# smallflyingpig/speech-to-image-translation-without-text

Measured on AMD Instinct MI355X. Metric: StackGAN-v2 3-stage G+D train-step images/sec at 256px, higher is better.
Workload: dtype f32

## Files before the change

### include/s2i_hip.h

```cpp
#ifndef S2I_HIP_H
#define S2I_HIP_H

#include <stddef.h>
#include <stdint.h>

#ifdef __cplusplus
extern "C" {
#endif

#define S2I_ABI_VERSION 7

#define S2I_CONV_K1      0
#define S2I_CONV_K3S1    1
#define S2I_CONV_K4S2    2
#define S2I_TCONV_K4S2   3

#define S2I_CONV_1D      4

#define S2I_ACT_NONE     0
#define S2I_ACT_GLU      1
#define S2I_ACT_LRELU    2
#define S2I_ACT_TANH     3
#define S2I_ACT_RELU     4

// ... 93 lines not shown


int s2i_conv_bf16_plan_query(const s2i_conv_desc* d, long long out[21]);
int s2i_pack_conv_weight_bf16(const s2i_conv_desc* d, const float* packed, int R, int C, unsigned short* out,
                              void* stream);
typedef struct s2i_pack16_item {
  const float* P;
  unsigned short* out;
  int R, C, kind, flip, transpose, T, nphase, Nn, Npad, Kk, CK, gx, gy, block0;
} s2i_pack16_item;
int s2i_pack16_item_fill(const s2i_conv_desc* d, const float* packed, int R, int C, unsigned short* out,
                         s2i_pack16_item* item);
int s2i_pack_conv_weights_bf16_batched(const s2i_pack16_item* items_dev, int n, int total_blocks, void* stream);
int s2i_conv_forward_bf16(const s2i_conv_desc* d, const unsigned short* x, const unsigned short* w,
                          const float* cls_bias, unsigned short* y, float* part, void* ws, size_t ws_bytes,
                          void* stream);
int s2i_conv_forward_dt(const s2i_conv_desc* d, const void* x, int x_dtype, const float* cvec, const float* w,
                        const float* bias, const float* cls_bias, void* y, int y_dtype, float* part, void* ws,
                        size_t ws_bytes, void* stream);
size_t s2i_wgrad_workspace_bytes_dt(const s2i_wgrad_desc* d, int a_dtype, int g_dtype);
int s2i_wgrad_plan_query(const s2i_wgrad_desc* d, int a_dtype, int g_dtype, int planes, int in_act, int out[12]);
int s2i_conv_wgrad_dt(const s2i_wgrad_desc* d, const void* a, int a_dtype, const float* cvec, const void* g,
                      int g_dtype, float* grad_oihw, void* ws, size_t ws_bytes, void* stream);
int s2i_bn_act_forward_dt(int dtype, const void* y, long long M, int groups, int C, const float* coef4, int act,
                          const void* residual, void* out, void* stream);
int s2i_bn_act_bwd_reduce_dt(int dtype, const void* y, const void* dout, int lddout, long long M, int groups, int C,
                             const float* coef4, int act, float* part, int nparts, void* stream);
int s2i_bn_act_bwd_apply_dt(int dtype, const void* y, const void* dout, int lddout, long long M, int groups, int C,
                            const float* coef4, const float* red2, int act, void* dy, void* stream);
int s2i_act_backward_dt(int dtype, const void* out, const void* dout, int lddout, long long M, int C, int act,
                        void* dy, void* stream);
int s2i_nchw_to_nhwc_dt(int dtype, const float* src, void* dst, int B, int C, int H, int W, int Cp, void* stream);
int s2i_nhwc_to_nchw_dt(int dtype, const void* src, int lds, float* dst, int B, int C, int H, int W, void* stream);
int s2i_spatial_sum_dt(int dtype, const void* src, int ld, int B, int HW, int C, float* dst, void* ws,
                       size_t ws_bytes, void* stream);
int s2i_tap_sums_dt(int dtype, const void* dy, int B, int H, int W, int C, float* tapsum, void* ws, size_t ws_bytes,
                    void* stream);
int s2i_cast(const void* src, int src_dtype, void* dst, int dst_dtype, long long n, void* stream);

int s2i_pack_conv_weight(const float* w_oihw, float* packed, int O, int I, int KH, int KW,
                         int Ip, int mode, void* stream);
typedef struct s2i_pack_item {
  const float* w;
  float* packed;
  int O, I, KH, KW, Ip, mode, gx, block0;
} s2i_pack_item;
// ... 227 lines not shown
```

### speech_to_image_translation_without_text_amd/_lib.py

```python
import ctypes
import os

import torch

_HERE = os.path.dirname(os.path.abspath(__file__))
LIB_PATH = os.path.join(_HERE, "libs2i_hip.so")

CONV_K1, CONV_K3S1, CONV_K4S2, TCONV_K4S2, CONV_1D = 0, 1, 2, 3, 4
ACT_NONE, ACT_GLU, ACT_LRELU, ACT_TANH, ACT_RELU = 0, 1, 2, 3, 4
PACK_PLAIN, PACK_UPFOLD = 0, 1
DT_F32, DT_BF16 = 0, 1
POOL_MAX3S2, POOL_AVG3S1, POOL_GLOBAL = 0, 1, 2
POOL_THEN_LRN, LRN_THEN_POOL = 0, 1
LOGMEL_BFT, LOGMEL_NHWC = 0, 1
ENC_LOSS_JEL, ENC_LOSS_L1, ENC_LOSS_DISTILL = 1, 2, 4
LOGMEL_TILE_FRAMES = 64
PCM_U8, PCM_S16, PCM_S24, PCM_S32, PCM_F32, PCM_F64 = 0, 1, 2, 3, 4, 5
RESAMPLE_TILE = 1024
RESAMPLE_MAX_WINDOW = 13826
TOPK_MAX = 64
RANK_GATHER, RANK_COUNT = 0, 1
DIFFAUG_COLOR, DIFFAUG_TRANSLATION, DIFFAUG_CUTOUT = 1, 2, 4
ABI_VERSION = 7
WGRAD_KERNELS = ("f32-128x128", "f32-128x64", "f32-128x32", "f32-64x64", "f32-256x128", "f32-256x256", "f32-96x64", "f32-96x32",
# ... 24 lines not shown
                                     "tile_rows", "in_act", "in_groups")]


class Conv2dDesc(ctypes.Structure):
    _fields_ = [(n, c_int) for n in ("B", "H", "W", "C", "ldx", "N", "kh", "kw", "sh", "sw", "ph", "pw", "Ho", "Wo",
                                     "ldy", "coff", "relu", "tile")]


class WgradDesc(ctypes.Structure):
    _fields_ = [(n, c_int) for n in ("kind", "B", "H", "W", "Ca", "Cc", "N", "ldg", "swap", "fold",
                                     "O", "I", "KH", "KW", "accumulate", "i_off", "I_total", "a_act", "a_groups")]


class PackItem(ctypes.Structure):
    _fields_ = [("w", c_void_p), ("packed", c_void_p)] + [(n, c_int) for n in ("O", "I", "KH", "KW", "Ip", "mode", "gx",
                                                                               "block0")]


class Pack16Item(ctypes.Structure):
    _fields_ = [("P", c_void_p), ("out", c_void_p)] + [(n, c_int) for n in (
        "R", "C", "kind", "flip", "transpose", "T", "nphase", "Nn", "Npad", "Kk", "CK", "gx", "gy", "block0")]


P = c_void_p
_SIGNATURES = {
    "s2i_last_error": (ctypes.c_char_p, []),
    "s2i_version": (c_int, []),
    "s2i_check_device": (c_int, []),
    "s2i_set_tuning": (c_int, [ctypes.c_char_p, c_int]),
    "s2i_get_tuning": (c_int, [ctypes.c_char_p, ctypes.POINTER(c_int)]),
    "s2i_conv_workspace_bytes": (c_size_t, [ctypes.POINTER(ConvDesc)]),
    "s2i_conv_stat_parts": (c_int, [ctypes.POINTER(ConvDesc)]),
    "s2i_conv_plan_query": (c_int, [ctypes.POINTER(ConvDesc), c_int, c_int, c_int, c_int, c_int, ctypes.POINTER(c_int * 15)]),
    "s2i_conv_forward": (c_int, [ctypes.POINTER(ConvDesc), P, P, P, P, P, P, P, c_size_t, P]),
    "s2i_conv_forward_cls": (c_int, [ctypes.POINTER(ConvDesc), P, P, P, P, P, P, P, P, c_size_t, P]),
    "s2i_conv_forward_in": (c_int, [ctypes.POINTER(ConvDesc), P, P, P, P, P, P, c_size_t, P]),
    "s2i_conv_wgrad_in_eligible": (c_int, [ctypes.POINTER(WgradDesc)]),
    "s2i_conv_wgrad_in": (c_int, [ctypes.POINTER(WgradDesc), P, P, P, P, P, c_size_t, P]),
    "s2i_conv_split_eligible": (c_int, [ctypes.POINTER(ConvDesc)]),
    "s2i_conv_forward_split": (c_int, [ctypes.POINTER(ConvDesc), P, P, P, c_int, c_int, c_int, P, P, P, P, P, c_size_t, P]),
    "s2i_split_packed_weight": (c_int, [P, c_int, c_int, c_int, c_int, P, P, P]),
    "s2i_wgrad_workspace_bytes_split": (c_size_t, [ctypes.POINTER(WgradDesc), c_int]),
    "s2i_conv_wgrad_split": (c_int, [ctypes.POINTER(WgradDesc), c_int, P, P, P, P, P, c_size_t, P]),
    "s2i_conv_bf16_plan_query": (c_int, [ctypes.POINTER(ConvDesc), ctypes.POINTER(c_ll * 21)]),
    "s2i_pack16_item_fill": (c_int, [ctypes.POINTER(ConvDesc), P, c_int, c_int, P, ctypes.POINTER(Pack16Item)]),
    "s2i_pack_conv_weights_bf16_batched": (c_int, [P, c_int, c_int, P]),
    "s2i_pack_conv_weight_bf16": (c_int, [ctypes.POINTER(ConvDesc), P, c_int, c_int, P, P]),
    "s2i_conv_forward_bf16": (c_int, [ctypes.POINTER(ConvDesc), P, P, P, P, P, P, c_size_t, P]),
    "s2i_conv_forward_dt": (c_int, [ctypes.POINTER(ConvDesc), P, c_int, P, P, P, P, P, c_int, P, P, c_size_t, P]),
    "s2i_wgrad_workspace_bytes_dt": (c_size_t, [ctypes.POINTER(WgradDesc), c_int, c_int]),
    "s2i_conv_wgrad_dt": (c_int, [ctypes.POINTER(WgradDesc), P, c_int, P, P, c_int, P, P, c_size_t, P]),
    "s2i_wgrad_plan_query": (c_int, [ctypes.POINTER(WgradDesc), c_int, c_int, c_int, c_int, ctypes.POINTER(c_int * 12)]),
    "s2i_bn_act_forward_dt": (c_int, [c_int, P, c_ll, c_int, c_int, P, c_int, P, P, P]),
    "s2i_bn_act_bwd_reduce_dt": (c_int, [c_int, P, P, c_int, c_ll, c_int, c_int, P, c_int, P, c_int, P]),
    "s2i_bn_act_bwd_apply_dt": (c_int, [c_int, P, P, c_int, c_ll, c_int, c_int, P, P, c_int, P, P]),
    "s2i_act_backward_dt": (c_int, [c_int, P, P, c_int, c_ll, c_int, c_int, P, P]),
    "s2i_nchw_to_nhwc_dt": (c_int, [c_int, P, P, c_int, c_int, c_int, c_int, c_int, P]),
    "s2i_nhwc_to_nchw_dt": (c_int, [c_int, P, c_int, P, c_int, c_int, c_int, c_int, P]),
    "s2i_spatial_sum_dt": (c_int, [c_int, P, c_int, c_int, c_int, c_int, P, P, c_size_t, P]),
    "s2i_tap_sums_dt": (c_int, [c_int, P, c_int, c_int, c_int, c_int, P, P, c_size_t, P]),
    "s2i_cast": (c_int, [P, c_int, P, c_int, c_ll, P]),
    "s2i_cvec_bias_table": (c_int, [P, P, c_int, c_int, c_int, c_int, c_int, P, P, c_size_t, P]),
    "s2i_border_sums_workspace_bytes": (c_size_t, [c_int, c_int, c_int, c_int]),
    "s2i_tap_sums": (c_int, [P, c_int, c_int, c_int, c_int, P, P, c_size_t, P]),
    "s2i_cvec_grads": (c_int, [P, P, P, c_int, c_int, c_int, c_int, c_int, c_int, c_int, P, P, c_int, P]),
    "s2i_wgrad_workspace_bytes": (c_size_t, [ctypes.POINTER(WgradDesc)]),
    "s2i_conv_wgrad": (c_int, [ctypes.POINTER(WgradDesc), P, P, P, P, P, c_size_t, P]),
    "s2i_pack_conv_weight": (c_int, [P, P, c_int, c_int, c_int, c_int, c_int, c_int, P]),
    "s2i_pack_conv_weights_batched": (c_int, [P, c_int, c_int, c_int, P]),
    "s2i_bn_finalize": (c_int, [P, c_int, c_int, c_int, c_ll, P, P, P, P, P, c_float, c_float, P, P]),
    "s2i_bn_eval_coeffs": (c_int, [c_int, P, P, P, P, c_float, P, P]),
    "s2i_bn_act_forward": (c_int, [P, c_ll, c_int, c_int, P, c_int, P, P, P]),
    "s2i_colstats": (c_int, [P, c_ll, c_int, c_int, P, c_int, P]),
    "s2i_bn_act_bwd_reduce": (c_int, [P, P, c_int, c_ll, c_int, c_int, P, c_int, P, c_int, P]),
    "s2i_bn_bwd_finalize": (c_int, [P, c_int, c_int, c_int, c_ll, P, P, c_int, P, P]),
# ... 195 lines not shown
```

### speech_to_image_translation_without_text_amd/csrc/s2i_wgrad.hip

```cpp
#include "s2i_igemm.h"

namespace {

struct WgradP {
  const float* __restrict__ a;
  const float* __restrict__ cvec;
  const float* __restrict__ g;
  float* __restrict__ slab;
  int B, H, W, Ca, Cc, Cin;
  int Ho, Wo, lgWo, lgHoWo;
  int M, N, ldg, K, T, kind;
  int cps, nchunks;
  int a16, g16;
  unsigned a_bytes, c_bytes, g_bytes;
  const float* __restrict__ a_coef;
  int a_groups, a_ipg;
};

__device__ __forceinline__ bool wgrad_col(const WgradP& p, int kcol, int kw, int& c, int& dy, int& dx) {
  c = 0;
  dy = 0;
  dx = 0;
  if (kcol >= p.K) return false;
  const int t = kcol / p.Cin;
// ... 540 lines not shown
    const f32x4 av0 = load_a(m0);
    load_g(m0, g0);
    fma9(av0, g0);
  }
#pragma unroll
  for (int t = 0; t < 9; ++t)
#pragma unroll
    for (int j = 0; j < 4; ++j) {
      f32x4 v = acc[t][j];
#pragma unroll
      for (int sft = LPP; sft < 64; sft <<= 1)
#pragma unroll
        for (int n = 0; n < 4; ++n) v[n] += __shfl_xor(v[n], sft);
      if (pl == 0) red[wave][(t * LPP + q) * 4 + j] = v;
    }
  __syncthreads();
  float* outp = p.slab + (size_t)blockIdx.x * p.K * 4;
  for (int e = tid; e < 9 * LPP * 4; e += 256) {
    const f32x4 v = red[0][e] + red[1][e] + red[2][e] + red[3][e];
    *reinterpret_cast<f32x4*>(outp + (size_t)e * 4) = v;
  }
}

__global__ __launch_bounds__(256) void slab_sum_tree_kernel(float* __restrict__ slab, int S, int n4) {
  __shared__ f32x4 sh[256];
  const int tid = threadIdx.x;
  const int e = blockIdx.x * 4 + (tid & 3), sl = tid >> 2;
  f32x4 v = {0.f, 0.f, 0.f, 0.f};
  if (e < n4)
    for (int s = sl; s < S; s += 64) v += *reinterpret_cast<const f32x4*>(slab + ((size_t)s * n4 + e) * 4);
  sh[tid] = v;
  __syncthreads();
  for (int h = 32; h >= 1; h >>= 1) {
    if (sl < h) sh[tid] += sh[tid + h * 4];
    __syncthreads();
  }
  if (sl == 0 && e < n4) *reinterpret_cast<f32x4*>(slab + (size_t)e * 4) = sh[tid];
}

__global__ __launch_bounds__(256) void slab_sum_kernel(float* __restrict__ slab, int S, long long n4) {
  for (long long e = (long long)blockIdx.x * blockDim.x + threadIdx.x; e < n4;
       e += (long long)gridDim.x * blockDim.x) {
    f32x4 v = *reinterpret_cast<const f32x4*>(slab + e * 4);
    for (int s = 1; s < S; ++s) v += *reinterpret_cast<const f32x4*>(slab + ((size_t)s * n4 + e) * 4);
    *reinterpret_cast<f32x4*>(slab + e * 4) = v;
  }
}

__global__ __launch_bounds__(256) void wgrad_finish_kernel(const float* __restrict__ slab, int S, int K, int N,
                                                           int Cg, int O, int I, int Tp, int T, int swap, int fold,
                                                           int accumulate, int RT, float* __restrict__ grad,
                                                           int i_off, int I_total) {
  extern __shared__ float tile[];
  const int tid = threadIdx.x;
  const int ncols = swap ? I : O, nrows = swap ? O : I;
  const int c0 = blockIdx.x * 32, r0 = blockIdx.y * RT;
  const size_t sstride = (size_t)K * N;
  const int nload = T * RT * 32;
  for (int e = tid; e < nload; e += 256) {
    const int c_l = e & 31;
    const int r_l = (e >> 5) % RT;
    const int t = (e >> 5) / RT;
    const int c = c0 + c_l, r = r0 + r_l;
    float v = 0.f;
    if (c < ncols && r < nrows) {
      const float* sp = slab + ((size_t)t * Cg + r) * N + c;
      for (int s = 0; s < S; ++s) v += sp[s * sstride];
    }
    tile[(t * RT + r_l) * 33 + c_l] = v;
  }
  __syncthreads();
  const int nout = 32 * RT * Tp;
  for (int w = tid; w < nout; w += 256) {
    const int tapo = w % Tp;
    const int rest = w / Tp;
    int o_l, i_l, r_l, c_l;
    if (swap) { i_l = rest & 31; o_l = rest >> 5; r_l = o_l; c_l = i_l; }
    else { i_l = rest % RT; o_l = rest / RT; r_l = i_l; c_l = o_l; }
    const int o = swap ? r0 + o_l : c0 + o_l;
    const int i = swap ? c0 + i_l : r0 + i_l;
    if (o >= O || i >= I) continue;
    float v;
    if (fold) {
      const int ky = tapo / 3, kx = tapo - ky * 3;
      v = 0.f;
#pragma unroll
      for (int ay = 0; ay < 2; ++ay)
#pragma unroll
        for (int ax = 0; ax < 2; ++ax) {
          const int t = ((2 - ky) + ay) * 4 + (2 - kx) + ax;
          v += tile[(t * RT + r_l) * 33 + c_l];
        }
    } else {
      v = tile[(tapo * RT + r_l) * 33 + c_l];
    }
    float* gp = grad + ((size_t)o * I_total + i_off + i) * Tp + tapo;
    *gp = accumulate ? *gp + v : v;
  }
}

}

template <int BM, int BN, int WM, int WN>
static void launch_wgrad_split(const WgradP& p, dim3 grid, int planes, hipStream_t st) {
  if (planes == 1) hipLaunchKernelGGL((igemm_wgrad_split_kernel<BM, BN, WM, WN, 1>), grid, dim3(256), 0, st, p);
  else if (planes == 2) hipLaunchKernelGGL((igemm_wgrad_split_kernel<BM, BN, WM, WN, 2>), grid, dim3(256), 0, st, p);
  else hipLaunchKernelGGL((igemm_wgrad_split_kernel<BM, BN, WM, WN, 3>), grid, dim3(256), 0, st, p);
}

static int launch_wgrad(const s2i_wgrad_desc* d, const WgPlan& pl, const float* a, const float* cvec, const float* g,
                        float* grad_oihw, void* ws, size_t ws_bytes, void* stream, int a16, int g16, const float* a_coef) {
  S2I_REQUIRE((a || d->Ca == 0) && g && grad_oihw, "wgrad: null operand");
  S2I_REQUIRE(d->Cc == 0 || cvec != nullptr, "wgrad: cvec is null but Cc > 0");
  const size_t need = wg_workspace_bytes(pl, d->N);
  S2I_REQUIRE(ws && ws_bytes >= need, "wgrad: workspace too small (%zu < %zu)", ws_bytes, need);
  hipStream_t st = (hipStream_t)stream;
  WgradP p;
  p.a = a; p.cvec = cvec; p.g = g; p.slab = (float*)ws;
  p.B = d->B; p.H = d->H; p.W = d->W; p.Ca = d->Ca; p.Cc = d->Cc; p.Cin = pl.Cin;
  p.Ho = pl.Ho; p.Wo = pl.Wo; p.lgWo = s2i_ilog2(pl.Wo); p.lgHoWo = s2i_ilog2(pl.Ho * pl.Wo);
  p.M = pl.M; p.N = d->N; p.ldg = d->ldg; p.K = pl.K; p.T = pl.T; p.kind = d->kind;
  p.cps = pl.cps; p.nchunks = pl.nchunks;
  p.a16 = a16; p.g16 = g16;
  p.a_coef = a_coef; p.a_groups = d->a_groups < 1 ? 1 : d->a_groups; p.a_ipg = d->B / p.a_groups;
  {
    const unsigned long long ab = (unsigned long long)d->B * d->H * d->W * d->Ca * (a16 ? 2ull : 4ull);
    const unsigned long long gb = (unsigned long long)pl.M * d->ldg * (g16 ? 2ull : 4ull);
    S2I_REQUIRE(ab < 0x7ff00000ull && gb < 0x7ff00000ull, "wgrad: tensor exceeds the 2 GiB buffer-addressing window");
    p.a_bytes = (unsigned)ab; p.g_bytes = (unsigned)gb;
    p.c_bytes = (unsigned)((unsigned long long)d->B * d->Cc * 4ull);
  }
  const dim3 grid(pl.gx, pl.gy, pl.gz);
#define WG_LAUNCH(id, ...) case id: hipLaunchKernelGGL((__VA_ARGS__), grid, dim3(pl.threads), 0, st, p); break
#define WG_LAUNCH_SPLIT(id, ...) case id: launch_wgrad_split<__VA_ARGS__>(p, grid, pl.planes, st); break
  switch (pl.kernel) {
    WG_LAUNCH(WG_F32_128x128, igemm_wgrad_kernel<128, 128, 2, 2>);
    WG_LAUNCH(WG_F32_128x64, igemm_wgrad_kernel<128, 64, 2, 2>);
// ... 8 lines not shown
    WG_LAUNCH(WG_B16_128x64, igemm_wgrad_b16_kernel<128, 64, 2, 2>);
    WG_LAUNCH(WG_B16_128x32, igemm_wgrad_b16_kernel<128, 32, 4, 1>);
    WG_LAUNCH(WG_B16_64x64, igemm_wgrad_b16_kernel<64, 64, 2, 2>);
    WG_LAUNCH(WG_B16_256x128, igemm_wgrad_b16_kernel<256, 128, 4, 2>);
    WG_LAUNCH(WG_B16_256x256, igemm_wgrad_b16_kernel<256, 256, 4, 4>);
    WG_LAUNCH(WG_B16D1_64x64, igemm_wgrad_b16_kernel<64, 64, 2, 2, true>);
    WG_LAUNCH_SPLIT(WG_SPLIT_128x128, 128, 128, 2, 2);
    WG_LAUNCH_SPLIT(WG_SPLIT_128x64, 128, 64, 2, 2);
    WG_LAUNCH_SPLIT(WG_SPLIT_128x32, 128, 32, 4, 1);
    WG_LAUNCH_SPLIT(WG_SPLIT_64x64, 64, 64, 2, 2);
    WG_LAUNCH(WG_ROWS3_32x64, wgrad_k3_rows_kernel<32, 64, 3, 1, 3>);
    WG_LAUNCH(WG_ROWS3_32x32, wgrad_k3_rows_kernel<32, 32, 3, 1, 3>);
    WG_LAUNCH(WG_ROWS3_64x128, wgrad_k3_rows_kernel<64, 128, 2, 2, 1>);
    WG_LAUNCH(WG_ROWS3_64x64, wgrad_k3_rows_kernel<64, 64, 2, 2, 1>);
    WG_LAUNCH(WG_ROWS3_64x32, wgrad_k3_rows_kernel<64, 32, 2, 1, 1>);
    WG_LAUNCH(WG_SMALLN_16, small_n_wgrad_kernel<4>);
    WG_LAUNCH(WG_SMALLN_32, small_n_wgrad_kernel<8>);
    WG_LAUNCH(WG_SMALLN_64, small_n_wgrad_kernel<16>);
    default: S2I_FAIL("wgrad: the plan names no kernel (%d)", (int)pl.kernel);
  }
#undef WG_LAUNCH
#undef WG_LAUNCH_SPLIT
  S2I_LAUNCH_CHECK("igemm_wgrad");
  {
    const int ncols = d->swap ? d->I : d->O, nrows = d->swap ? d->O : d->I;
    int RT = 8;
    while (RT > 1 && (long long)s2i_cdiv(ncols, 32) * s2i_cdiv(nrows, RT) < 128) RT >>= 1;
    dim3 fgrid(s2i_cdiv(ncols, 32), s2i_cdiv(nrows, RT));
    const size_t shb = (size_t)pl.T * RT * 33 * sizeof(float);
    int S = pl.slabs;
    const long long kn = (long long)pl.K * d->N;
    if (pl.kernel >= WG_SMALLN_16 || (S >= 32 && (kn % 4) == 0 && kn / 4 < (1 << 18))) {
      hipLaunchKernelGGL(slab_sum_tree_kernel, dim3(s2i_cdiv(kn / 4, 4)), dim3(256), 0, st, (float*)ws, S, (int)(kn / 4));
      S2I_LAUNCH_CHECK("slab_sum_tree");
      S = 1;
    } else if (S > 2 && (kn % 4) == 0) {
      int sb = s2i_cdiv(kn / 4, 256);
      if (sb > 4096) sb = 4096;
      hipLaunchKernelGGL(slab_sum_kernel, dim3(sb), dim3(256), 0, st, (float*)ws, S, kn / 4);
      S2I_LAUNCH_CHECK("slab_sum");
      S = 1;
    }
    hipLaunchKernelGGL(wgrad_finish_kernel, fgrid, dim3(256), shb, st, (const float*)ws, S, pl.K, d->N,
                       pl.Cin, d->O, d->I, d->KH * d->KW, pl.T, d->swap, d->fold, d->accumulate, RT, grad_oihw,
                       d->i_off, d->I_total > 0 ? d->I_total : d->I);
  }
  S2I_LAUNCH_CHECK("wgrad_finish");
  return 0;
}

static int conv_wgrad_impl(const s2i_wgrad_desc* d, int planes, const float* a, const float* cvec, const float* g,
                           float* grad_oihw, void* ws, size_t ws_bytes, void* stream, int a16 = 0, int g16 = 0, const float* a_coef = nullptr) {
  WgMode mode;
  WgPlan pl;
  if (wg_mode(a16, g16, planes, a_coef != nullptr, &mode) || plan_wgrad(d, mode, &pl)) return 1;
  return launch_wgrad(d, pl, a, cvec, g, grad_oihw, ws, ws_bytes, stream, a16, g16, a_coef);
}

extern "C" int s2i_conv_wgrad_in(const s2i_wgrad_desc* d, const float* a_raw, const float* a_coef, const float* g,
                                 float* grad_oihw, void* ws, size_t ws_bytes, void* stream) {
  S2I_REQUIRE(a_coef != nullptr, "wgrad(apply-on-load): null coefficient table");
  return conv_wgrad_impl(d, 0, a_raw, nullptr, g, grad_oihw, ws, ws_bytes, stream, 0, 0, a_coef);
}

extern "C" int s2i_conv_wgrad_dt(const s2i_wgrad_desc* d, const void* a, int a_dtype, const float* cvec, const void* g,
                                 int g_dtype, float* grad_oihw, void* ws, size_t ws_bytes, void* stream) {
  S2I_REQUIRE((a_dtype == S2I_DT_F32 || a_dtype == S2I_DT_BF16) && (g_dtype == S2I_DT_F32 || g_dtype == S2I_DT_BF16),
              "wgrad: unknown dtype");
  return conv_wgrad_impl(d, 0, (const float*)a, cvec, (const float*)g, grad_oihw, ws, ws_bytes, stream,
                         a_dtype == S2I_DT_BF16, g_dtype == S2I_DT_BF16);
}

extern "C" int s2i_conv_wgrad(const s2i_wgrad_desc* d, const float* a, const float* cvec, const float* g,
                              float* grad_oihw, void* ws, size_t ws_bytes, void* stream) {
  return conv_wgrad_impl(d, 0, a, cvec, g, grad_oihw, ws, ws_bytes, stream);
}

extern "C" int s2i_conv_wgrad_split(const s2i_wgrad_desc* d, int planes, const float* a, const float* cvec,
                                    const float* g, float* grad_oihw, void* ws, size_t ws_bytes, void* stream) {
  S2I_REQUIRE(planes >= 1 && planes <= 3, "wgrad(split): need 1 to 3 bf16 planes");
  return conv_wgrad_impl(d, planes, a, cvec, g, grad_oihw, ws, ws_bytes, stream);
// ... 2 lines not shown
```

### speech_to_image_translation_without_text_amd/ops.py

```python
import ctypes
import os

import torch

from . import _lib
from ._lib import (ACT_GLU, ACT_LRELU, ACT_NONE, CONV_K1, CONV_K3S1, CONV_K4S2, DT_BF16, DT_F32,
                   PACK_PLAIN, PACK_UPFOLD, TCONV_K4S2, ConvDesc, WgradDesc, check, ptr, stream)

BN_EPS = 1e-5
BN_MOMENTUM = 0.1

DIRECT_PARAM_GRAD = False


def _direct(p):
    return (DIRECT_PARAM_GRAD and p is not None and p.requires_grad and p.grad is not None
            and p.grad.is_contiguous())


class param_grad_mode:

    def __init__(self, direct=True):
        self.new = bool(direct)

# ... 19 lines not shown

    def __init__(self):
        self.buf = {}
        self.pinned = False
        self.retired = []

    def get(self, nbytes, device):
        nbytes = max(int(nbytes), 16)
        key = (device, stream())
        cur = self.buf.get(key)
        if cur is None or cur.numel() * 4 < nbytes:
            if cur is not None and self.pinned:
                self.retired.append(cur)
            cur = torch.empty((nbytes + 3) // 4 + 1024, dtype=torch.float32, device=device)
            self.buf[key] = cur
        return cur


_ws = _Workspace()


def pin_graph_resources():
    _ws.pinned = True


def invalidate_derived(params):
    for p in params:
        packs = getattr(p, '_s2i_packs', None)
        if packs:
            for ent in packs.values():
                ent[0]._s2i_gen = getattr(ent[0], '_s2i_gen', 0) + 1


def _roundup4(v):
    return (v + 3) & ~3


def packed_weight(w, mode=0):
    packs = getattr(w, '_s2i_packs', None)
    if packs is None:
        packs = {}
        w._s2i_packs = packs
    ent = packs.get(mode)
    ver, addr = w._version, w.data_ptr()
    if ent is not None and ent[1] == ver and ent[2] == addr and ent[0].device == w.device:
        return ent[0]
# ... 227 lines not shown
    check(lib.s2i_conv_forward_dt(ctypes.byref(d), ptr(x), _dt(x), None, ptr(packed) + 4 * int(w_offset), ptr(bias),
                                  ptr(cls_bias), ptr(y), _dt(y), ptr(part), ptr(ws), ws.numel() * 4, stream()),
          "s2i_conv_forward_dt")
    return y, part, nparts


def wgrad_any(kind, a, g, grad_shape, *, swap=0, fold=0, out=None, accumulate=False, i_off=0, I_total=0):
    lib = _lib_ready()
    B, H, W, Ca = a.shape
    N = g.shape[-1]
    if len(grad_shape) == 2:
        O, I, KH, KW = grad_shape[0], grad_shape[1], 1, 1
    else:
        O, I, KH, KW = grad_shape
    d = WgradDesc(kind, B, H, W, Ca, 0, N, N, swap, fold, O, I, KH, KW, 1 if accumulate else 0, i_off, I_total)
    if EXEC_LOG is not None:
        Ho, Wo = _geom(kind, H, W)
        _log_exec("wgrad%s k%d a[%d,%d,%d,%d] g%d" % ("16" if a.dtype == g.dtype == torch.bfloat16 else "", kind, B, H, W,
                                                      Ca, N), B * Ho * Wo, N, _TAPS[kind] * Ca, a.numel(), g.numel(),
                  _TAPS[kind] * Ca * N, a.element_size(), 4)
    if out is None:
        full = grad_shape if not I_total else (O, I_total, KH, KW)
        out = torch.empty(full, dtype=torch.float32, device=a.device)
    wsb = lib.s2i_wgrad_workspace_bytes_dt(ctypes.byref(d), _dt(a), _dt(g))
    if wsb == 0:
        check(1, "s2i_wgrad_workspace_bytes_dt")
    ws = _ws.get(wsb, a.device)
    check(lib.s2i_conv_wgrad_dt(ctypes.byref(d), ptr(a), _dt(a), None, ptr(g), _dt(g), ptr(out), ptr(ws), ws.numel() * 4,
                                stream()), "s2i_conv_wgrad_dt")
    return out


EXEC_LOG = None
_TAPS = {CONV_K1: 1, CONV_K3S1: 9, CONV_K4S2: 16, TCONV_K4S2: 4}


def _log_exec(what, M, N, K, in_elems, w_elems, out_elems, esize_in=4, esize_out=4):
    if EXEC_LOG is not None:
        EXEC_LOG.append((what, 2.0 * M * N * K, in_elems * esize_in + w_elems * esize_in + out_elems * esize_out, M, N, K))


def _geom(kind, H, W):
    if kind == CONV_K4S2:
        return H // 2, W // 2
    if kind == TCONV_K4S2:
        return 2 * H, 2 * W
    return H, W


TILE_ROWS = 0


DEFER_ACT = os.environ.get("S2I_DEFER_ACT", "0") == "1"
# ... 69 lines not shown


def wgrad_raw(kind, a, cvec, g, grad_shape, *, swap=0, fold=0, out=None, accumulate=False, i_off=0, I_total=0, a_src=None,
              g_cols=None):
    lib = _lib_ready()
    B, H, W, Ca = a.shape
    Cc = 0 if cvec is None else cvec.shape[1]
    N = g.shape[-1]
    if g_cols is not None:
        return _wgrad_cols(kind, a, g, grad_shape, g_cols)
    if len(grad_shape) == 2:
        O, I, KH, KW = grad_shape[0], grad_shape[1], 1, 1
    else:
        O, I, KH, KW = grad_shape
    d = WgradDesc(kind, B, H, W, Ca, Cc, N, N, swap, fold, O, I, KH, KW, 1 if accumulate else 0, i_off, I_total,
                  a_src.act if a_src is not None else 0, a_src.groups if a_src is not None else 0)
    if EXEC_LOG is not None:
        Ho, Wo = _geom(kind, H, W)
        _log_exec("wgrad k%d a[%d,%d,%d,%d+%d] g%d" % (kind, B, H, W, Ca, Cc, N), B * Ho * Wo, N, _TAPS[kind] * (Ca + Cc),
                  a.numel(), g.numel(), _TAPS[kind] * (Ca + Cc) * N)
    if out is None:
        full = grad_shape if not I_total else (O, I_total, KH, KW)
        out = torch.empty(full, dtype=torch.float32, device=a.device)
    if a_src is not None:
        wsb = lib.s2i_wgrad_workspace_bytes(ctypes.byref(d))
        if wsb == 0:
            check(1, "s2i_wgrad_workspace_bytes")
        ws = _ws.get(wsb, a.device)
        check(lib.s2i_conv_wgrad_in(ctypes.byref(d), ptr(a), ptr(a_src.coef), ptr(g), ptr(out), ptr(ws), ws.numel() * 4,
                                    stream()), "s2i_conv_wgrad_in")
        return out
    if MATH_PLANES:
        wsb = lib.s2i_wgrad_workspace_bytes_split(ctypes.byref(d), MATH_PLANES)
        if wsb == 0:
            check(1, "s2i_wgrad_workspace_bytes_split")
        ws = _ws.get(wsb, a.device)
        check(lib.s2i_conv_wgrad_split(ctypes.byref(d), MATH_PLANES, ptr(a), ptr(cvec), ptr(g), ptr(out), ptr(ws),
                                       ws.numel() * 4, stream()), "s2i_conv_wgrad_split")
        return out
    wsb = lib.s2i_wgrad_workspace_bytes(ctypes.byref(d))
    if wsb == 0:
        check(1, "s2i_wgrad_workspace_bytes")
    ws = _ws.get(wsb, a.device)
    check(lib.s2i_conv_wgrad(ctypes.byref(d), ptr(a), ptr(cvec), ptr(g), ptr(out), ptr(ws), ws.numel() * 4,
                             stream()), "s2i_conv_wgrad")
    return out
# ... 1364 lines not shown
```

### speech_to_image_translation_without_text_amd/trainer.py

```python
import json
import os
import time
from copy import deepcopy

import numpy as np
import torch
import torch.nn as nn

from . import ops
from ._lib import S2IError
from .miscc.config import cfg
from .miscc.utils import mkdir_p
from .model import D_NET64, D_NET128, D_NET256, D_NET512, D_NET1024, G_NET, INCEPTION_V3


def compute_mean_covariance(img):
    batch_size, channel_num, height, width = img.shape
    num_pixels = height * width
    mu = img.mean(2, keepdim=True).mean(3, keepdim=True)
    img_hat = (img - mu.expand_as(img)).view(batch_size, channel_num, num_pixels)
    covariance = torch.bmm(img_hat, img_hat.transpose(1, 2)) / num_pixels
    return mu, covariance


# ... 265 lines not shown
class condGANTrainer(object):
    d_overlap_min = 1 << 20

    def __init__(self, output_dir, data_loader, imsize, my_dataset_flag, local_rank=0, distributed=False):
        self.my_dataset_flag = my_dataset_flag
        if output_dir is not None:
            if not cfg.TRAIN.FLAG:
                output_dir += "_eval"
            self.model_dir = os.path.join(output_dir, 'Model')
            self.image_dir = os.path.join(output_dir, 'Image')
            self.log_dir = os.path.join(output_dir, 'Log')
            for d in (self.model_dir, self.image_dir, self.log_dir):
                mkdir_p(d)
        self.gpus = [local_rank]
        self.batch_size = cfg.TRAIN.BATCH_SIZE
        self.max_epoch = cfg.TRAIN.MAX_EPOCH
        self.snapshot_interval = cfg.TRAIN.SNAPSHOT_INTERVAL
        self.data_loader = data_loader
        self.num_batches = len(data_loader) if data_loader is not None else 0
        self.distributed = distributed
        self.world = torch.distributed.get_world_size() if distributed else 1
        self._pending = []
        self.stack_d_passes = True
        self.d_streams = os.environ.get("S2I_D_STREAMS", "1") == "1" and torch.cuda.is_available()
        self._side_streams = None
        self._graph = None
        self._labels_dev = None
        self._g_pass = []
        self._aug = None
        if os.environ.get("S2I_GRAPH", "0") == "1":
            self.enable_graph()
        self.inception_model = None
        self.inception_min_batches = 500
        self._inception_rows = []
        if cfg.TRAIN.INCEPTION_WEIGHTS:
            self.enable_inception(cfg.TRAIN.INCEPTION_WEIGHTS)
        self.fixed_noise = self.fixed_eps = None

    def _make_d_streams(self):
        key = (torch.cuda.current_device(), self.num_Ds)
        if key not in _D_STREAMS:
            _D_STREAMS[key] = [torch.cuda.Stream() for i in range(self.num_Ds)]
        return _D_STREAMS[key]

    def build(self, netG=None, netsD=None, start_count=0):
        if netG is None:
# ... 136 lines not shown
            key = (str(dev), float(u))
            if getattr(self, '_bce_consts', (None,))[0] != key:
                self._bce_consts = (key, torch.tensor([1., 1., 0., 1., 0., 0.], device=dev),
                                    torch.tensor([1., u, 1., u, 1., u], device=dev))
            return ops.BCEMulti.apply(self._bce_consts[1], self._bce_consts[2], 3, *self._stacked_logits)
        errD_real = ops.BCELoss.apply(real_logits[0], 1.0, 1.0)
        errD_wrong = ops.BCELoss.apply(wrong_logits[0], 0.0, 1.0)
        errD_fake = ops.BCELoss.apply(fake_logits[0], 0.0, 1.0)
        if len(real_logits) > 1 and u > 0:
            errD_real = errD_real + ops.BCELoss.apply(real_logits[1], 1.0, u)
            errD_wrong = errD_wrong + ops.BCELoss.apply(wrong_logits[1], 1.0, u)
            errD_fake = errD_fake + ops.BCELoss.apply(fake_logits[1], 0.0, u)
            return errD_real + errD_wrong + errD_fake
        return errD_real + 0.5 * (errD_wrong + errD_fake)

    def train_Dnet(self, idx, count, defer_step=False):
        flat = self.flatsD[idx]
        flat.zero_grad()
        split = getattr(self, '_d_split', [None] * self.num_Ds)[idx] if self.distributed else None
        if split is not None:
            self._d_tail_work[idx], self._d_fires[idx] = None, 0
            self._d_hook_armed[idx] = True
        errD = self._d_loss(idx)
        errD.backward()
        if split is not None:
            self._d_hook_armed[idx] = False
        if split is not None and self._d_tail_work[idx] is not None:
            works = [self._reduce_async(flat, 0, split), self._d_tail_work[idx]]
            self._d_tail_work[idx] = None
        else:
            works = [self._reduce_async(flat)]
        if defer_step:
            self._pending.append((flat, works))
        else:
            for work in works:
                if work is not None:
                    work.wait()
            flat.adam(1.0 / self.world)
        return errD

    def _flush_d_steps(self):
        for flat, works in self._pending:
            for work in works:
                if work is not None:
                    work.wait()
            flat.adam(1.0 / self.world)
        self._pending = []
# ... 30 lines not shown
            grads.append(g_fake)
            if g_mu is not None:
                g_mu_total = g_mu if g_mu_total is None else g_mu_total + g_mu
        self._g_pass = [None] * self.num_Ds
        extra = 0
        if cfg.TRAIN.COEFF.COLOR_LOSS > 0:
            coef = cfg.TRAIN.COEFF.COLOR_LOSS
            for hi, lo in ((-1, -2), (-2, -3)):
                if self.num_Ds >= -lo:
                    mu1, cov1 = compute_mean_covariance(self.fake_imgs[hi])
                    mu2, cov2 = compute_mean_covariance(self.fake_imgs[lo].detach())
                    extra = extra + coef * nn.functional.mse_loss(mu1, mu2) + coef * 5 * nn.functional.mse_loss(cov1, cov2)
        kl_loss = KL_loss(self.mu, self.logvar) * cfg.TRAIN.COEFF.KL
        own = kl_loss + extra
        errG_total = errG_total + own.detach()
        if g_mu_total is not None:
            roots.append(self.mu)
            grads.append(g_mu_total)
        roots.append(own)
        grads.append(torch.ones_like(own))
        split = getattr(self, '_g_split', None) if self.distributed else None
        self._g_tail_work = None
        self._g_hook_armed = split is not None
        torch.autograd.backward(roots, grads)
        self._g_hook_armed = False
        if self.distributed and self._g_tail_work is not None:
            work = self._reduce_async(self.flatG, 0, split)
            work.wait()
            self._g_tail_work.wait()
            self._g_tail_work = None
        else:
            work = self._reduce_async(self.flatG)
            if work is not None:
                work.wait()
        self.flatG.adam(1.0 / self.world)
        return kl_loss.detach(), errG_total

    def train_Gnet(self, count):
        self._labels_dev = None
        self._g_pass = [None] * self.num_Ds
        main = torch.cuda.current_stream() if self.d_streams else None
        if self.d_streams and self._side_streams is None:
            self._side_streams = self._make_d_streams()
        for i in range(self.num_Ds):
            if self.d_streams:
                self._side_streams[i].wait_stream(main)
                with torch.cuda.stream(self._side_streams[i]):
# ... 412 lines not shown
```

Baseline: 784.3.

## Batch weight-gradient slab reduce and finish kernels across a backward pass

Weight-gradient GEMMs now write their partial slabs into a per-optimizer arena, and the slab reduction and finish (layout/accumulate) steps are deferred. At the end of each backward pass they run as two batched kernels driven by a device-side item table. The aim is to replace many small reduce and finish launches per layer with two launches, cutting launch overhead and idle gaps. In exchange it adds arena memory, overlap tracking that forces early flushes, and uploads of cached tables. All finish blocks also share the largest LDS size.

```diff
diff --git a/include/s2i_hip.h b/include/s2i_hip.h
--- a/include/s2i_hip.h
+++ b/include/s2i_hip.h
@@ -139,6 +139,26 @@
 int s2i_wgrad_plan_query(const s2i_wgrad_desc* d, int a_dtype, int g_dtype, int planes, int in_act, int out[12]);
 int s2i_conv_wgrad_dt(const s2i_wgrad_desc* d, const void* a, int a_dtype, const float* cvec, const void* g,
                       int g_dtype, float* grad_oihw, void* ws, size_t ws_bytes, void* stream);
+
+#define S2I_WGRAD_REDUCE_NONE 0
+#define S2I_WGRAD_REDUCE_STREAM 1
+#define S2I_WGRAD_REDUCE_TREE 2
+typedef struct s2i_wgrad_finish_item {
+  float* slab;
+  float* grad;
+  int S, S_fin;
+  int reduce;
+  int K, N, Cin, O, I, Tp, T, swap, fold, accumulate;
+  int RT;
+  int i_off, I_total;
+  int red_block0, red_blocks;
+  int fin_block0, fin_gx, fin_gy;
+} s2i_wgrad_finish_item;
+int s2i_conv_wgrad_slabs(const s2i_wgrad_desc* d, const void* a, int a_dtype, const float* cvec, const void* g,
+                         int g_dtype, int planes, float* grad_oihw, void* slabs, size_t slab_bytes,
+                         s2i_wgrad_finish_item* item_out, void* stream);
+int s2i_conv_wgrad_finish_batched(const s2i_wgrad_finish_item* items_dev, int n, int red_blocks_total,
+                                  int fin_blocks_total, size_t max_finish_lds_bytes, void* stream);
 int s2i_bn_act_forward_dt(int dtype, const void* y, long long M, int groups, int C, const float* coef4, int act,
                           const void* residual, void* out, void* stream);
 int s2i_bn_act_bwd_reduce_dt(int dtype, const void* y, const void* dout, int lddout, long long M, int groups, int C,
diff --git a/speech_to_image_translation_without_text_amd/_lib.py b/speech_to_image_translation_without_text_amd/_lib.py
--- a/speech_to_image_translation_without_text_amd/_lib.py
+++ b/speech_to_image_translation_without_text_amd/_lib.py
@@ -70,6 +70,21 @@
         "R", "C", "kind", "flip", "transpose", "T", "nphase", "Nn", "Npad", "Kk", "CK", "gx", "gy", "block0")]
 
 
+WGRAD_REDUCE_NONE, WGRAD_REDUCE_STREAM, WGRAD_REDUCE_TREE = 0, 1, 2
+WGRAD_FINISH_FIELDS = ("S", "S_fin", "reduce", "K", "N", "Cin", "O", "I", "Tp", "T", "swap", "fold", "accumulate", "RT",
+                       "i_off", "I_total", "red_block0", "red_blocks", "fin_block0", "fin_gx", "fin_gy")
+
+
+class WgradFinishItem(ctypes.Structure):
+    _fields_ = [("slab", c_void_p), ("grad", c_void_p)] + [(n, c_int) for n in WGRAD_FINISH_FIELDS]
+
+    def key(self):
+        return (self.slab, self.grad) + tuple(getattr(self, n) for n in WGRAD_FINISH_FIELDS)
+
+    def finish_lds_bytes(self):
+        return self.T * self.RT * 33 * 4
+
+
 P = c_void_p
 _SIGNATURES = {
     "s2i_last_error": (ctypes.c_char_p, []),
@@ -99,6 +114,9 @@
     "s2i_wgrad_workspace_bytes_dt": (c_size_t, [ctypes.POINTER(WgradDesc), c_int, c_int]),
     "s2i_conv_wgrad_dt": (c_int, [ctypes.POINTER(WgradDesc), P, c_int, P, P, c_int, P, P, c_size_t, P]),
     "s2i_wgrad_plan_query": (c_int, [ctypes.POINTER(WgradDesc), c_int, c_int, c_int, c_int, ctypes.POINTER(c_int * 12)]),
+    "s2i_conv_wgrad_slabs": (c_int, [ctypes.POINTER(WgradDesc), P, c_int, P, P, c_int, c_int, P, P, c_size_t,
+                                     ctypes.POINTER(WgradFinishItem), P]),
+    "s2i_conv_wgrad_finish_batched": (c_int, [P, c_int, c_int, c_int, c_size_t, P]),
     "s2i_bn_act_forward_dt": (c_int, [c_int, P, c_ll, c_int, c_int, P, c_int, P, P, P]),
     "s2i_bn_act_bwd_reduce_dt": (c_int, [c_int, P, P, c_int, c_ll, c_int, c_int, P, c_int, P, c_int, P]),
     "s2i_bn_act_bwd_apply_dt": (c_int, [c_int, P, P, c_int, c_ll, c_int, c_int, P, P, c_int, P, P]),
diff --git a/speech_to_image_translation_without_text_amd/csrc/s2i_wgrad.hip b/speech_to_image_translation_without_text_amd/csrc/s2i_wgrad.hip
--- a/speech_to_image_translation_without_text_amd/csrc/s2i_wgrad.hip
+++ b/speech_to_image_translation_without_text_amd/csrc/s2i_wgrad.hip
@@ -586,10 +586,10 @@
   }
 }
 
-__global__ __launch_bounds__(256) void slab_sum_tree_kernel(float* __restrict__ slab, int S, int n4) {
-  __shared__ f32x4 sh[256];
+
+__device__ __forceinline__ void slab_sum_tree_body(int bx, float* __restrict__ slab, int S, int n4, f32x4* sh) {
   const int tid = threadIdx.x;
-  const int e = blockIdx.x * 4 + (tid & 3), sl = tid >> 2;
+  const int e = bx * 4 + (tid & 3), sl = tid >> 2;
   f32x4 v = {0.f, 0.f, 0.f, 0.f};
   if (e < n4)
     for (int s = sl; s < S; s += 64) v += *reinterpret_cast<const f32x4*>(slab + ((size_t)s * n4 + e) * 4);
@@ -602,23 +602,29 @@
   if (sl == 0 && e < n4) *reinterpret_cast<f32x4*>(slab + (size_t)e * 4) = sh[tid];
 }
 
-__global__ __launch_bounds__(256) void slab_sum_kernel(float* __restrict__ slab, int S, long long n4) {
-  for (long long e = (long long)blockIdx.x * blockDim.x + threadIdx.x; e < n4;
-       e += (long long)gridDim.x * blockDim.x) {
+__global__ __launch_bounds__(256) void slab_sum_tree_kernel(float* __restrict__ slab, int S, int n4) {
+  __shared__ f32x4 sh[256];
+  slab_sum_tree_body(blockIdx.x, slab, S, n4, sh);
+}
+
+__device__ __forceinline__ void slab_sum_body(int bx, int nb, float* __restrict__ slab, int S, long long n4) {
+  for (long long e = (long long)bx * 256 + threadIdx.x; e < n4; e += (long long)nb * 256) {
     f32x4 v = *reinterpret_cast<const f32x4*>(slab + e * 4);
     for (int s = 1; s < S; ++s) v += *reinterpret_cast<const f32x4*>(slab + ((size_t)s * n4 + e) * 4);
     *reinterpret_cast<f32x4*>(slab + e * 4) = v;
   }
 }
 
-__global__ __launch_bounds__(256) void wgrad_finish_kernel(const float* __restrict__ slab, int S, int K, int N,
-                                                           int Cg, int O, int I, int Tp, int T, int swap, int fold,
-                                                           int accumulate, int RT, float* __restrict__ grad,
-                                                           int i_off, int I_total) {
-  extern __shared__ float tile[];
+__global__ __launch_bounds__(256) void slab_sum_kernel(float* __restrict__ slab, int S, long long n4) {
+  slab_sum_body(blockIdx.x, gridDim.x, slab, S, n4);
+}
+
+__device__ __forceinline__ void wgrad_finish_body(int bx, int by, const float* __restrict__ slab, int S, int K, int N, int Cg,
+                                                  int O, int I, int Tp, int T, int swap, int fold, int accumulate, int RT,
+                                                  float* __restrict__ grad, int i_off, int I_total, float* tile) {
   const int tid = threadIdx.x;
   const int ncols = swap ? I : O, nrows = swap ? O : I;
-  const int c0 = blockIdx.x * 32, r0 = blockIdx.y * RT;
+  const int c0 = bx * 32, r0 = by * RT;
   const size_t sstride = (size_t)K * N;
   const int nload = T * RT * 32;
   for (int e = tid; e < nload; e += 256) {
@@ -663,6 +669,38 @@
   }
 }
 
+__global__ __launch_bounds__(256) void wgrad_finish_kernel(const float* __restrict__ slab, int S, int K, int N,
+                                                           int Cg, int O, int I, int Tp, int T, int swap, int fold,
+                                                           int accumulate, int RT, float* __restrict__ grad,
+                                                           int i_off, int I_total) {
+  extern __shared__ float tile[];
+  wgrad_finish_body(blockIdx.x, blockIdx.y, slab, S, K, N, Cg, O, I, Tp, T, swap, fold, accumulate, RT, grad, i_off, I_total,
+                    tile);
+}
+
+__global__ __launch_bounds__(256) void wgrad_reduce_batched_kernel(const s2i_wgrad_finish_item* __restrict__ items, int n) {
+  __shared__ f32x4 sh[256];
+  int k = 0;
+  while (k + 1 < n && (int)blockIdx.x >= items[k + 1].red_block0) ++k;
+  const s2i_wgrad_finish_item it = items[k];
+  const int local = blockIdx.x - it.red_block0;
+  if (local < 0 || local >= it.red_blocks) return;
+  const long long n4 = (long long)it.K * it.N / 4;
+  if (it.reduce == S2I_WGRAD_REDUCE_TREE) slab_sum_tree_body(local, it.slab, it.S, (int)n4, sh);
+  else if (it.reduce == S2I_WGRAD_REDUCE_STREAM) slab_sum_body(local, it.red_blocks, it.slab, it.S, n4);
+}
+
+__global__ __launch_bounds__(256) void wgrad_finish_batched_kernel(const s2i_wgrad_finish_item* __restrict__ items, int n) {
+  extern __shared__ float tile[];
+  int k = 0;
+  while (k + 1 < n && (int)blockIdx.x >= items[k + 1].fin_block0) ++k;
+  const s2i_wgrad_finish_item it = items[k];
+  const int local = blockIdx.x - it.fin_block0;
+  if (local < 0 || local >= it.fin_gx * it.fin_gy) return;
+  wgrad_finish_body(local % it.fin_gx, local / it.fin_gx, it.slab, it.S_fin, it.K, it.N, it.Cin, it.O, it.I, it.Tp, it.T, it.swap,
+                    it.fold, it.accumulate, it.RT, it.grad, it.i_off, it.I_total, tile);
+}
+
 }
 
 template <int BM, int BN, int WM, int WN>
@@ -672,11 +710,10 @@
   else hipLaunchKernelGGL((igemm_wgrad_split_kernel<BM, BN, WM, WN, 3>), grid, dim3(256), 0, st, p);
 }
 
-static int launch_wgrad(const s2i_wgrad_desc* d, const WgPlan& pl, const float* a, const float* cvec, const float* g,
-                        float* grad_oihw, void* ws, size_t ws_bytes, void* stream, int a16, int g16, const float* a_coef) {
-  S2I_REQUIRE((a || d->Ca == 0) && g && grad_oihw, "wgrad: null operand");
+static int launch_wgrad_gemm(const s2i_wgrad_desc* d, const WgPlan& pl, const float* a, const float* cvec, const float* g,
+                             void* ws, size_t ws_bytes, size_t need, void* stream, int a16, int g16, const float* a_coef) {
+  S2I_REQUIRE((a || d->Ca == 0) && g, "wgrad: null operand");
   S2I_REQUIRE(d->Cc == 0 || cvec != nullptr, "wgrad: cvec is null but Cc > 0");
-  const size_t need = wg_workspace_bytes(pl, d->N);
   S2I_REQUIRE(ws && ws_bytes >= need, "wgrad: workspace too small (%zu < %zu)", ws_bytes, need);
   hipStream_t st = (hipStream_t)stream;
   WgradP p;
@@ -731,29 +768,62 @@
 #undef WG_LAUNCH
 #undef WG_LAUNCH_SPLIT
   S2I_LAUNCH_CHECK("igemm_wgrad");
-  {
-    const int ncols = d->swap ? d->I : d->O, nrows = d->swap ? d->O : d->I;
-    int RT = 8;
-    while (RT > 1 && (long long)s2i_cdiv(ncols, 32) * s2i_cdiv(nrows, RT) < 128) RT >>= 1;
-    dim3 fgrid(s2i_cdiv(ncols, 32), s2i_cdiv(nrows, RT));
-    const size_t shb = (size_t)pl.T * RT * 33 * sizeof(float);
-    int S = pl.slabs;
-    const long long kn = (long long)pl.K * d->N;
-    if (pl.kernel >= WG_SMALLN_16 || (S >= 32 && (kn % 4) == 0 && kn / 4 < (1 << 18))) {
-      hipLaunchKernelGGL(slab_sum_tree_kernel, dim3(s2i_cdiv(kn / 4, 4)), dim3(256), 0, st, (float*)ws, S, (int)(kn / 4));
-      S2I_LAUNCH_CHECK("slab_sum_tree");
-      S = 1;
-    } else if (S > 2 && (kn % 4) == 0) {
-      int sb = s2i_cdiv(kn / 4, 256);
-      if (sb > 4096) sb = 4096;
-      hipLaunchKernelGGL(slab_sum_kernel, dim3(sb), dim3(256), 0, st, (float*)ws, S, kn / 4);
-      S2I_LAUNCH_CHECK("slab_sum");
-      S = 1;
-    }
-    hipLaunchKernelGGL(wgrad_finish_kernel, fgrid, dim3(256), shb, st, (const float*)ws, S, pl.K, d->N,
-                       pl.Cin, d->O, d->I, d->KH * d->KW, pl.T, d->swap, d->fold, d->accumulate, RT, grad_oihw,
-                       d->i_off, d->I_total > 0 ? d->I_total : d->I);
-  }
+  return 0;
+}
+
+static void fill_finish_item(const s2i_wgrad_desc* d, const WgPlan& pl, void* ws, float* grad_oihw, s2i_wgrad_finish_item* it) {
+  const int ncols = d->swap ? d->I : d->O, nrows = d->swap ? d->O : d->I;
+  int RT = 8;
+  while (RT > 1 && (long long)s2i_cdiv(ncols, 32) * s2i_cdiv(nrows, RT) < 128) RT >>= 1;
+  it->slab = (float*)ws;
+  it->grad = grad_oihw;
+  it->S = it->S_fin = pl.slabs;
+  it->reduce = S2I_WGRAD_REDUCE_NONE;
+  it->red_block0 = it->red_blocks = 0;
+  const long long kn = (long long)pl.K * d->N;
+  if (pl.kernel >= WG_SMALLN_16 || (pl.slabs >= 32 && (kn % 4) == 0 && kn / 4 < (1 << 18))) {
+    it->reduce = S2I_WGRAD_REDUCE_TREE;
+    it->red_blocks = s2i_cdiv(kn / 4, 4);
+    it->S_fin = 1;
+  } else if (pl.slabs > 2 && (kn % 4) == 0) {
+    int sb = s2i_cdiv(kn / 4, 256);
+    if (sb > 4096) sb = 4096;
+    it->reduce = S2I_WGRAD_REDUCE_STREAM;
+    it->red_blocks = sb;
+    it->S_fin = 1;
+  }
+  it->K = pl.K; it->N = d->N; it->Cin = pl.Cin; it->O = d->O; it->I = d->I; it->Tp = d->KH * d->KW; it->T = pl.T;
+  it->swap = d->swap; it->fold = d->fold; it->accumulate = d->accumulate; it->RT = RT;
+  it->i_off = d->i_off; it->I_total = d->I_total > 0 ? d->I_total : d->I;
+  it->fin_block0 = 0;
+  it->fin_gx = s2i_cdiv(ncols, 32);
+  it->fin_gy = s2i_cdiv(nrows, RT);
+}
+
+static inline size_t finish_lds_bytes(const s2i_wgrad_finish_item& it) { return (size_t)it.T * it.RT * 33 * sizeof(float); }
+
+static int launch_slab_reduce(const s2i_wgrad_finish_item& it, hipStream_t st) {
+  if (it.reduce == S2I_WGRAD_REDUCE_TREE) {
+    hipLaunchKernelGGL(slab_sum_tree_kernel, dim3(it.red_blocks), dim3(256), 0, st, it.slab, it.S, (int)((long long)it.K * it.N / 4));
+    S2I_LAUNCH_CHECK("slab_sum_tree");
+  } else if (it.reduce == S2I_WGRAD_REDUCE_STREAM) {
+    hipLaunchKernelGGL(slab_sum_kernel, dim3(it.red_blocks), dim3(256), 0, st, it.slab, it.S, (long long)it.K * it.N / 4);
+    S2I_LAUNCH_CHECK("slab_sum");
+  }
+  return 0;
+}
+
+static int launch_wgrad(const s2i_wgrad_desc* d, const WgPlan& pl, const float* a, const float* cvec, const float* g,
+                        float* grad_oihw, void* ws, size_t ws_bytes, void* stream, int a16, int g16, const float* a_coef) {
+  S2I_REQUIRE(grad_oihw, "wgrad: null operand");
+  if (launch_wgrad_gemm(d, pl, a, cvec, g, ws, ws_bytes, wg_workspace_bytes(pl, d->N), stream, a16, g16, a_coef)) return 1;
+  hipStream_t st = (hipStream_t)stream;
+  s2i_wgrad_finish_item it;
+  fill_finish_item(d, pl, ws, grad_oihw, &it);
+  if (launch_slab_reduce(it, st)) return 1;
+  hipLaunchKernelGGL(wgrad_finish_kernel, dim3(it.fin_gx, it.fin_gy), dim3(256), finish_lds_bytes(it), st, (const float*)it.slab,
+                     it.S_fin, it.K, it.N, it.Cin, it.O, it.I, it.Tp, it.T, it.swap, it.fold, it.accumulate, it.RT, it.grad,
+                     it.i_off, it.I_total);
   S2I_LAUNCH_CHECK("wgrad_finish");
   return 0;
 }
@@ -766,6 +836,42 @@
   return launch_wgrad(d, pl, a, cvec, g, grad_oihw, ws, ws_bytes, stream, a16, g16, a_coef);
 }
 
+extern "C" int s2i_conv_wgrad_slabs(const s2i_wgrad_desc* d, const void* a, int a_dtype, const float* cvec, const void* g,
+                                    int g_dtype, int planes, float* grad_oihw, void* slabs, size_t slab_bytes,
+                                    s2i_wgrad_finish_item* item_out, void* stream) {
+  S2I_REQUIRE((a_dtype == S2I_DT_F32 || a_dtype == S2I_DT_BF16) && (g_dtype == S2I_DT_F32 || g_dtype == S2I_DT_BF16),
+              "wgrad: unknown dtype");
+  S2I_REQUIRE(item_out, "wgrad(slabs): null item");
+  const int a16 = a_dtype == S2I_DT_BF16, g16 = g_dtype == S2I_DT_BF16;
+  WgMode mode;
+  WgPlan pl;
+  if (wg_mode(a16, g16, planes, false, &mode) || plan_wgrad(d, mode, &pl)) return 1;
+  if (!slabs && slab_bytes == 0) {
+    fill_finish_item(d, pl, nullptr, grad_oihw, item_out);
+    return 0;
+  }
+  S2I_REQUIRE(grad_oihw, "wgrad(slabs): null operand");
+  const size_t need = (size_t)pl.slabs * pl.K * d->N * sizeof(float);
+  if (launch_wgrad_gemm(d, pl, (const float*)a, cvec, (const float*)g, slabs, slab_bytes, need, stream, a16, g16, nullptr)) return 1;
+  fill_finish_item(d, pl, slabs, grad_oihw, item_out);
+  return 0;
+}
+
+extern "C" int s2i_conv_wgrad_finish_batched(const s2i_wgrad_finish_item* items_dev, int n, int red_blocks_total,
+                                             int fin_blocks_total, size_t max_finish_lds_bytes, void* stream) {
+  S2I_REQUIRE(items_dev && n > 0 && red_blocks_total >= 0 && fin_blocks_total > 0, "wgrad(batched finish): bad args");
+  S2I_REQUIRE(max_finish_lds_bytes > 0 && max_finish_lds_bytes <= (size_t)16 * 8 * 33 * sizeof(float),
+              "wgrad(batched finish): %zu bytes of LDS (at most 16 taps x 8 rows)", max_finish_lds_bytes);
+  hipStream_t st = (hipStream_t)stream;
+  if (red_blocks_total > 0) {
+    hipLaunchKernelGGL(wgrad_reduce_batched_kernel, dim3(red_blocks_total), dim3(256), 0, st, items_dev, n);
+    S2I_LAUNCH_CHECK("wgrad_reduce_batched");
+  }
+  hipLaunchKernelGGL(wgrad_finish_batched_kernel, dim3(fin_blocks_total), dim3(256), max_finish_lds_bytes, st, items_dev, n);
+  S2I_LAUNCH_CHECK("wgrad_finish_batched");
+  return 0;
+}
+
 extern "C" int s2i_conv_wgrad_in(const s2i_wgrad_desc* d, const float* a_raw, const float* a_coef, const float* g,
                                  float* grad_oihw, void* ws, size_t ws_bytes, void* stream) {
   S2I_REQUIRE(a_coef != nullptr, "wgrad(apply-on-load): null coefficient table");
diff --git a/speech_to_image_translation_without_text_amd/ops.py b/speech_to_image_translation_without_text_amd/ops.py
--- a/speech_to_image_translation_without_text_amd/ops.py
+++ b/speech_to_image_translation_without_text_amd/ops.py
@@ -1,5 +1,6 @@
 import ctypes
 import os
+import weakref
 
 import torch
 
@@ -65,6 +66,8 @@
 
 def pin_graph_resources():
     _ws.pinned = True
+    for arena in _wgrad_arenas:
+        arena.pinned = True
 
 
 def invalidate_derived(params):
@@ -338,6 +341,8 @@
     if out is None:
         full = grad_shape if not I_total else (O, I_total, KH, KW)
         out = torch.empty(full, dtype=torch.float32, device=a.device)
+    if _wgrad_route(lib, d, a, _dt(a), None, g, _dt(g), 0, out, accumulate, True, "s2i_conv_wgrad_slabs"):
+        return out
     wsb = lib.s2i_wgrad_workspace_bytes_dt(ctypes.byref(d), _dt(a), _dt(g))
     if wsb == 0:
         check(1, "s2i_wgrad_workspace_bytes_dt")
@@ -345,6 +350,162 @@
     check(lib.s2i_conv_wgrad_dt(ctypes.byref(d), ptr(a), _dt(a), None, ptr(g), _dt(g), ptr(out), ptr(ws), ws.numel() * 4,
                                 stream()), "s2i_conv_wgrad_dt")
     return out
+
+
+_WGRAD_SCOPE = None
+_wgrad_arenas = weakref.WeakSet()
+_wgrad_tables = {}
+_wgrad_need = {}
+WGRAD_STATS = {"batched": 0, "deferred": 0, "immediate": 0, "uploads": 0}
+
+
+class _WgradArena:
+
+    def __init__(self):
+        self.buf, self.off, self.left, self.total = None, 0, [], 0
+        self.pinned = torch.cuda.is_available() and torch.cuda.is_current_stream_capturing()
+        _wgrad_arenas.add(self)
+
+    def take(self, nbytes, device, scope):
+        n = (int(nbytes) // 4 + 63) & ~63
+        self.total += n
+        if self.buf is None or self.off + n > self.buf.numel():
+            if self.buf is not None and self.pinned:
+                if n > self.buf.numel():
+                    return None
+                scope.flush()
+            else:
+                if self.buf is not None:
+                    self.left.append(self.buf)
+                self.buf = torch.empty(max(n, 2 * self.buf.numel() if self.buf is not None else 0), dtype=torch.float32,
+                                       device=device)
+                self.off = 0
+        p = self.buf.data_ptr() + 4 * self.off
+        self.off += n
+        return p
+
+    def rewind(self):
+        moved = bool(self.left)
+        if not self.pinned and self.buf is not None and self.total > self.buf.numel():
+            self.buf = torch.empty(self.total, dtype=torch.float32, device=self.buf.device)
+            moved = True
+        self.left, self.off, self.total = [], 0, 0
+        return moved
+
+
+def _wgrad_table(items, device):
+    red0 = fin0 = lds = 0
+    for it in items:
+        it.red_block0, it.fin_block0 = red0, fin0
+        red0 += it.red_blocks
+        fin0 += it.fin_gx * it.fin_gy
+        lds = max(lds, it.finish_lds_bytes())
+    key = tuple(it.key() for it in items)
+    tab = _wgrad_tables.get(key)
+    if tab is None:
+        arr = (_lib.WgradFinishItem * len(items))(*items)
+        tab = torch.frombuffer(bytearray(bytes(arr)), dtype=torch.uint8).to(device)
+        WGRAD_STATS["uploads"] += 1
+        while len(_wgrad_tables) > 64 and not _ws.pinned:
+            del _wgrad_tables[next(iter(_wgrad_tables))]
+        _wgrad_tables[key] = tab
+    return tab, red0, fin0, lds
+
+
+class batched_wgrad_finish:
+
+    def __init__(self, flat):
+        self.flat = flat
+        self.items, self.ranges, self.sizes, self.groups = [], [], [], []
+        self.lo = flat.g.data_ptr()
+        self.hi = self.lo + 4 * flat.g.numel()
+        arena = getattr(flat, '_s2i_wgrad_arena', None)
+        if arena is None:
+            arena = flat._s2i_wgrad_arena = _WgradArena()
+        self.arena = arena
+
+    def __enter__(self):
+        global _WGRAD_SCOPE
+        self.old = _WGRAD_SCOPE
+        _WGRAD_SCOPE = self
+        return self
+
+    def __exit__(self, *exc):
+        global _WGRAD_SCOPE
+        _WGRAD_SCOPE = self.old
+        if exc[0] is None:
+            self.flush()
+        self.items, self.ranges, self.sizes = [], [], []
+        if self.arena.rewind() and exc[0] is None:
+            for group in self.groups:
+                off, moved = 0, []
+                for it, n in group:
+                    it = _lib.WgradFinishItem.from_buffer_copy(it)
+                    it.slab = self.arena.buf.data_ptr() + 4 * off
+                    off += n
+                    moved.append(it)
+                _wgrad_table(moved, self.flat.g.device)
+        self.groups = []
+        return False
+
+    def covers(self, out, accumulate):
+        return (out is not None and accumulate and out.is_contiguous()
+                and self.lo <= out.data_ptr() and out.data_ptr() + 4 * out.numel() <= self.hi)
+
+    def settle(self, out, i_off=0, I=0, I_total=0):
+        if out is None or not self.items:
+            return
+        lo = out.data_ptr()
+        hi = lo + 4 * out.numel()
+        for (plo, phi, pi_off, pI, pI_total) in self.ranges:
+            if plo < hi and lo < phi:
+                if plo == lo and I_total and pI_total == I_total and (pi_off + pI <= i_off or i_off + I <= pi_off):
+                    continue
+                self.flush()
+                return
+
+    def defer(self, lib, d, a, a_dt, cvec, g, g_dt, planes, out, what):
+        key = (tuple(getattr(d, f) for f, _ in d._fields_), a_dt, g_dt, planes)
+        need = _wgrad_need.get(key)
+        if need is None:
+            q = _lib.WgradFinishItem()
+            check(lib.s2i_conv_wgrad_slabs(ctypes.byref(d), None, a_dt, None, None, g_dt, planes, None, None, 0, ctypes.byref(q),
+                                           None), what)
+            need = _wgrad_need[key] = 4 * q.S * q.K * q.N
+        self.settle(out, d.i_off, d.I, d.I_total)
+        slab = self.arena.take(need, out.device, self)
+        if slab is None:
+            return False
+        item = _lib.WgradFinishItem()
+        check(lib.s2i_conv_wgrad_slabs(ctypes.byref(d), ptr(a), a_dt, ptr(cvec), ptr(g), g_dt, planes, ptr(out), slab, need,
+                                       ctypes.byref(item), stream()), what)
+        self.items.append(item)
+        self.sizes.append((need // 4 + 63) & ~63)
+        self.ranges.append((out.data_ptr(), out.data_ptr() + 4 * out.numel(), d.i_off, d.I, d.I_total))
+        WGRAD_STATS["deferred"] += 1
+        return True
+
+    def flush(self):
+        items, sizes, self.items, self.ranges, self.sizes = self.items, self.sizes, [], [], []
+        self.arena.off = 0
+        if not items:
+            return
+        self.groups.append(list(zip(items, sizes)))
+        tab, red0, fin0, lds = _wgrad_table(items, self.flat.g.device)
+        check(_lib_ready().s2i_conv_wgrad_finish_batched(ptr(tab), len(items), red0, fin0, lds, stream()),
+              "s2i_conv_wgrad_finish_batched")
+        WGRAD_STATS["batched"] += 1
+
+
+def _wgrad_route(lib, d, a, a_dt, cvec, g, g_dt, planes, out, accumulate, deferrable, what):
+    sc = _WGRAD_SCOPE
+    if sc is None:
+        return False
+    if deferrable and sc.covers(out, accumulate) and sc.defer(lib, d, a, a_dt, cvec, g, g_dt, planes, out, what):
+        return True
+    sc.settle(out)
+    WGRAD_STATS["immediate"] += 1
+    return False
 
 
 EXEC_LOG = None
@@ -460,6 +621,8 @@
     if out is None:
         full = grad_shape if not I_total else (O, I_total, KH, KW)
         out = torch.empty(full, dtype=torch.float32, device=a.device)
+    if _wgrad_route(lib, d, a, DT_F32, cvec, g, DT_F32, MATH_PLANES, out, accumulate, a_src is None, "s2i_conv_wgrad_slabs"):
+        return out
     if a_src is not None:
         wsb = lib.s2i_wgrad_workspace_bytes(ctypes.byref(d))
         if wsb == 0:
diff --git a/speech_to_image_translation_without_text_amd/trainer.py b/speech_to_image_translation_without_text_amd/trainer.py
--- a/speech_to_image_translation_without_text_amd/trainer.py
+++ b/speech_to_image_translation_without_text_amd/trainer.py
@@ -311,6 +311,7 @@
         self.world = torch.distributed.get_world_size() if distributed else 1
         self._pending = []
         self.stack_d_passes = True
+        self.batch_wgrad = os.environ.get("S2I_BATCH_WGRAD", "1") == "1"
         self.d_streams = os.environ.get("S2I_D_STREAMS", "1") == "1" and torch.cuda.is_available()
         self._side_streams = None
         self._graph = None
@@ -493,7 +494,11 @@
             self._d_tail_work[idx], self._d_fires[idx] = None, 0
             self._d_hook_armed[idx] = True
         errD = self._d_loss(idx)
-        errD.backward()
+        if self.batch_wgrad and split is None:
+            with ops.batched_wgrad_finish(flat):
+                errD.backward()
+        else:
+            errD.backward()
         if split is not None:
             self._d_hook_armed[idx] = False
         if split is not None and self._d_tail_work[idx] is not None:
@@ -570,7 +575,11 @@
         split = getattr(self, '_g_split', None) if self.distributed else None
         self._g_tail_work = None
         self._g_hook_armed = split is not None
-        torch.autograd.backward(roots, grads)
+        if self.batch_wgrad and split is None:
+            with ops.batched_wgrad_finish(self.flatG):
+                torch.autograd.backward(roots, grads)
+        else:
+            torch.autograd.backward(roots, grads)
         self._g_hook_armed = False
         if self.distributed and self._g_tail_work is not None:
             work = self._reduce_async(self.flatG, 0, split)
```

Result: no change. 787.7, median of 6 (+0.4%).
